# RuihanGao/visual-tactile-synthesis

Hardware: AMD Instinct MI355X
Metric: train_images_per_sec (higher is better)
Workload: dtype f32; 1 GPU; skitG G+D1+D2 train step, 1024x1024 sketch->(RGB,tactile), 4 images/GPU, 64 tactile patches/image, LPIPS/CLIP terms off (no weights offline); global_batch=4, parallelism=dp1, losses_finite=True, hip_graph=True, d2_visualisation_pass=True, train_only=False, full=False

## Files before the change

visual-tactile-synthesis_amd/csrc/vts_conv.hip:

```cpp
#include "vts_conv_kernel.h"

thread_local int t_stat_spl = 0;

namespace {

__global__ __launch_bounds__(256) void conv_split_epilogue_kernel(const ConvK p, int KS) {
  const int co = blockIdx.y, n = blockIdx.z;
  const int64_t oplane = (int64_t)p.OH * p.OW;
  const int64_t o = (int64_t)blockIdx.x * 256 + threadIdx.x;
  if (o >= oplane) return;
  float v = 0.f;
  for (int ks = 0; ks < KS; ++ks) v += p.part[(((int64_t)ks * p.N + n) * p.Cout + co) * oplane + o];
  v += p.bias ? p.bias[co] : 0.f;
  if (p.act_out == VTS_ACT_TANH) v = tanhf(v);
  if (p.dm) {
    const float dsc = p.dmsc ? p.dmsc[n * p.dmC + co] : 1.f, dsh = p.dmsh ? p.dmsh[n * p.dmC + co] : 0.f;
    v *= vts_act_grad(p.dm[n * p.dmns + co * oplane + o] * dsc + dsh, p.dm_act);
  }
  float* ob = p.out + n * p.ons + co * oplane + o;
  *ob = p.accumulate ? *ob + v : v;
}

struct InStatsOut {
  float *scale, *shift, *mean, *rstd;
// ... 143 lines not shown
  VTS_CHECK_ARG(d->stride == 1 || d->stride == 2, "vts_conv4x4: stride %d unsupported", d->stride);
  VTS_CHECK_ARG(d->Cout >= 1, "vts_conv4x4: Cout %d", d->Cout);
  if (d->Cout > 80) {
    for (int c0 = 0; c0 < d->Cout; c0 += 80) {
      vts_conv_desc g = *d;
      const int64_t oplane = (int64_t)d->OH * d->OW;
      g.Cout = d->Cout - c0 < 80 ? d->Cout - c0 : 80;
      g.w = d->w + (int64_t)c0 * d->ws_co;
      g.bias = d->bias ? d->bias + c0 : nullptr;
      g.out = d->out + c0 * oplane;
      if (d->dmask.data) {
        g.dmask.data = d->dmask.data + c0 * oplane;
        g.dmask.scale = d->dmask.scale ? d->dmask.scale + c0 : nullptr;
        g.dmask.shift = d->dmask.shift ? d->dmask.shift + c0 : nullptr;
      }
      const int rc = conv4x4_impl(&g, stream, nullptr, nullptr, StatWs{nullptr, 0});
      if (rc != VTS_OK) return rc;
    }
    return VTS_OK;
  }
  VTS_CHECK_ARG(d->N >= 1 && d->IH >= 1 && d->IW >= 1 && d->OH >= 1 && d->OW >= 1, "vts_conv4x4: bad shape");
  VTS_CHECK_ARG(d->in0.C >= 1 && d->in1.C >= 0, "vts_conv4x4: bad channel counts");
  VTS_CHECK_ARG(d->OH <= d->IH * d->stride + 16 && d->OW <= d->IW * d->stride + 16 && d->pad >= -8 && d->pad <= 8,
                "vts_conv4x4: output %dx%d / pad %d implausible for input %dx%d s%d", d->OH, d->OW, d->pad, d->IH, d->IW, d->stride);
  VTS_CHECK_ARG(d->pad_dx >= -8 && d->pad_dx <= 8 && !(d->transposed && d->stride == 2 && d->pad_dx != 0), "vts_conv4x4: bad pad_dx %d", d->pad_dx);
  if (d->transposed && d->stride == 2) {
    VTS_CHECK_ARG((d->OH + 2 * d->pad - 4) / d->stride + 1 == d->IH && (d->OW + 2 * d->pad - 4) / d->stride + 1 == d->IW && d->pad >= 0,
                  "vts_conv4x4: transposed output %dx%d inconsistent with input %dx%d s%d p%d", d->OH, d->OW, d->IH,
                  d->IW, d->stride, d->pad);
  }
  {
    const int rh0 = vts_conv_head_try(d, (hipStream_t)stream);
    if (rh0 != VTS_ERR_UNSUPPORTED) return rh0;
    static const int use_small = vts_tune_set("VTS_NO_SMALL") ? 0 : 1;
    if (use_small) {
      const int rc = vts_conv_small_try(d, (hipStream_t)stream);
      if (rc != VTS_ERR_UNSUPPORTED) return rc;
    }
  }
  ConvK k;
  k.s0 = d->in0.data; k.sc0 = d->in0.scale; k.sh0 = d->in0.shift; k.ns0 = d->in0.nstride; k.C0 = d->in0.C;
  k.s1 = d->in1.data; k.sc1 = d->in1.scale; k.sh1 = d->in1.shift; k.ns1 = d->in1.nstride;
  k.C1 = d->in1.data ? d->in1.C : 0;
  k.Cin = k.C0 + k.C1;
  k.IH = d->IH; k.IW = d->IW; k.OH = d->OH; k.OW = d->OW; k.Cout = d->Cout; k.pad = d->pad; k.padx = d->pad + d->pad_dx;
  k.w = d->w; k.ws_co = d->ws_co; k.ws_ci = d->ws_ci; k.bias = d->bias;
  k.out = d->out; k.ons = d->out_nstride;
  k.act_in = d->act_in; k.act_out = d->act_out;
  k.dm = d->dmask.data; k.dmsc = d->dmask.scale; k.dmsh = d->dmask.shift; k.dmns = d->dmask.nstride;
  k.dm_act = d->dmask_act; k.dmC = d->dmask.C;
  k.accumulate = d->accumulate;
  k.N = d->N; k.CG = 1; k.cps = 1 << 30; k.part = nullptr; k.tiles_x = 0; k.stat_part = nullptr; k.stat_spl = 0; k.bsum_part = nullptr;
#ifdef VTS_PROFILING
  static const int ablate = vts_tune("VTS_ABLATE", 0);
  k.ablate = ablate;
  k.trace = nullptr;
#endif
  static const int xcd_swizzle = vts_tune("VTS_XCD_SWIZZLE", 1);
  k.xcd_swizzle = xcd_swizzle;
  static const int direct_epi = vts_tune("VTS_DIRECT_EPI", 1);
  k.direct_epi = direct_epi && (int64_t)d->Cout * d->OH * d->OW * 4 < (int64_t)OOB_OFF && (!d->dmask.data || (int64_t)d->dmask.C * d->OH * d->OW * 4 < (int64_t)OOB_OFF);
  k.ident = vts_ident();
  VTS_CHECK_ARG(k.ident, "vts_conv4x4: could not allocate the identity constants");
  {
    const int64_t wfl = (int64_t)(d->Cout - 1) * d->ws_co + (int64_t)(k.Cin - 1) * d->ws_ci + 16;
    VTS_CHECK_ARG(wfl * 4 < (int64_t)OOB_OFF && (int64_t)d->IH * d->IW * 4 < (int64_t)OOB_OFF, "vts_conv4x4: tensor too large for 30-bit buffer offsets");
    k.wbytes = (int)(wfl * 4);
  }
  k.slope_in = vts_slope(d->act_in);
  k.identity_in = (d->act_in == VTS_ACT_NONE && !d->in0.scale && !d->in0.shift && !(d->in1.data && (d->in1.scale || d->in1.shift))) ? 1 : 0;
  hipStream_t st = (hipStream_t)stream;
  const int nr = (d->Cout + 15) / 16;
  const int N = d->N;
  static const int fuse_stats = vts_tune("VTS_FUSE_STATS", 1);
  const bool stats_ok = nd && fused && sw.p && fuse_stats && d->act_out == VTS_ACT_NONE && !d->dmask.data && !d->accumulate &&
                        nd->x == d->out && nd->N == N && nd->C == d->Cout && nd->HW == d->OH * d->OW && nd->nstride == d->out_nstride;
  const bool want_stats = stats_ok && k.direct_epi && sw.floats >= vts_conv4x4_norm_ws_floats(d);
  static const int fuse_bsums = vts_tune("VTS_FUSE_BSUMS", 1);
  const bool bsums_ok = bsums && fused && sw.p && fuse_bsums && d->act_out == VTS_ACT_NONE && d->dmask.data;
  const bool want_bsums = bsums_ok && k.direct_epi && sw.floats >= vts_conv4x4_norm_ws_floats(d);
  {
    int spl = 0;
    const int rc = vts_conv_px_try(d, st, stats_ok ? sw.p : nullptr, (!stats_ok && bsums_ok) ? sw.p : nullptr, sw.floats, &spl);
    if (rc != VTS_ERR_UNSUPPORTED) {
      if (rc == VTS_OK && spl > 0) *fused = 2 + spl;
      return rc;
    }
    const int rt = vts_conv_thin_try(d, st);
    if (rt != VTS_ERR_UNSUPPORTED) return rt;
  }
  {
    int rw, mt;
    full_tile(d->transposed, d->stride, nr, rw, mt);
    const bool ph4 = d->transposed && d->stride == 2;
    const int GH = ph4 ? (d->OH + 1) / 2 : d->OH, GW = ph4 ? (d->OW + 1) / 2 : d->OW;
    const int full_wgs = cdiv(GW, 16 * mt) * cdiv(GH, 4 * rw) * N;
    static const int split_ck = vts_tune("VTS_SPLIT_CK", 8);
    int ck = 4;
    const int nchunks = (k.Cin + 3) / 4;
    static const int small_thr = vts_tune("VTS_SMALL_WGS", 300);
    static const int target_wgs = vts_tune("VTS_TARGET_WGS", 256);
    if (full_wgs < small_thr && (nr > 1 || nchunks >= 8)) {
      const int base = cdiv(GW, 32) * cdiv(GH, 4) * N * nr;
      int KS = target_wgs / base;
      if (KS > nchunks / 2) KS = nchunks / 2;
      if (KS < 1) KS = 1;
      int cps = cdiv(nchunks, KS);
      KS = cdiv(nchunks, cps);
      const int64_t need = (int64_t)KS * N * d->Cout * d->OH * d->OW;
      if (KS > 1 && (!d->ws || d->ws_floats < need)) { KS = 1; cps = nchunks; }
      if (split_ck == 8 && k.Cin >= 32 && cps >= 4 && (cps % 2 == 0 || KS == 1)) { ck = 8; cps = (cps + 1) / 2; }
      k.CG = nr; k.cps = cps; k.part = KS > 1 ? d->ws : nullptr;
      const bool cg_stats = want_stats && KS == 1;
      if (cg_stats) k.stat_part = sw.p;
      const bool cg_bsums = want_bsums && KS == 1;
      if (cg_bsums) k.bsum_part = sw.p;
      int rc;
      if (!d->transposed) rc = d->stride == 2 ? vts_conv_split_m0s2(k, N, st, nr, KS, ck) : vts_conv_split_m0s1(k, N, st, nr, KS, ck);
      else rc = d->stride == 2 ? vts_conv_split_m1s2(k, N, st, nr, KS, ck) : vts_conv_split_m1s1(k, N, st, nr, KS, ck);
      if (rc == VTS_OK && (cg_stats || cg_bsums)) *fused = 2 + t_stat_spl;
      if (rc != VTS_OK || KS == 1) return rc;
      static const int fuse_in = vts_tune("VTS_FUSE_SPLIT_IN", 1);
      if (nd && nd->mode == 0 && fuse_in && (int64_t)d->OH * d->OW <= 4096 && d->act_out == VTS_ACT_NONE && !d->dmask.data && !d->accumulate &&
          nd->x == d->out && nd->N == N && nd->C == d->Cout && nd->HW == d->OH * d->OW && nd->nstride == d->out_nstride) {
        const InStatsOut q{nd->scale, nd->shift, nd->mean_out, nd->rstd_out, nd->eps};
        hipLaunchKernelGGL(conv_split_epilogue_in_kernel, dim3(N * d->Cout), dim3(256), 0, st, k, KS, q);
        VTS_CHECK_LAUNCH("vts_conv4x4 split epilogue + instance norm");
        vts_set_kernel("conv4x4_kernel<%d, %d, 1, 1, 2, %d, false, 0>+ksplit+in", d->transposed ? 1 : 0, d->stride, ck);
        *fused = 1;
        return VTS_OK;
      }
      static const int fuse_inbwd = vts_tune("VTS_FUSE_SPLIT_INBWD", 1);
      if (bsums && in_bwd_ok && fused && fuse_inbwd && (int64_t)d->OH * d->OW <= 4096 && d->act_out == VTS_ACT_NONE && d->dmask.data && d->dmask.scale &&
          d->dmask.shift && d->dmask.C == d->Cout) {
        hipLaunchKernelGGL(conv_split_epilogue_inbwd_kernel, dim3(N * d->Cout), dim3(256), 0, st, k, KS);
        VTS_CHECK_LAUNCH("vts_conv4x4 split epilogue + instance norm backward");
        vts_set_kernel("conv4x4_kernel<%d, %d, 1, 1, 2, %d, false, 0>+ksplit+inbwd", d->transposed ? 1 : 0, d->stride, ck);
        *fused = -1;
        return VTS_OK;
      }
      hipLaunchKernelGGL(conv_split_epilogue_kernel, dim3((unsigned)cdiv64((int64_t)d->OH * d->OW, 256), d->Cout, N), dim3(256), 0, st, k, KS);
      VTS_CHECK_LAUNCH("vts_conv4x4 split epilogue");
      return VTS_OK;
    }
  }
  if (want_stats) k.stat_part = sw.p;
  if (want_bsums) k.bsum_part = sw.p;
  const int rc = dispatch_full(d, k, nr, N, st);
  if (rc != VTS_OK || !(want_stats || want_bsums)) return rc;
  *fused = 2 + t_stat_spl;
  return VTS_OK;
}

static int dispatch_full(const vts_conv_desc* d, const ConvK& k, int nr, int N, hipStream_t st) {
  if (!d->transposed) return d->stride == 2 ? vts_conv_full_m0s2(k, nr, N, st) : vts_conv_full_m0s1(k, nr, N, st);
  return d->stride == 2 ? vts_conv_full_m1s2(k, nr, N, st) : vts_conv_full_m1s1(k, nr, N, st);
}
```

visual-tactile-synthesis_amd/csrc/vts_conv_kernel.h:

```cpp
#pragma once
#include <stdio.h>
#include <stdlib.h>
#include <string.h>

#include "vts_internal.h"

struct ConvK {
  const float *s0, *s1, *sc0, *sh0, *sc1, *sh1;
  int64_t ns0, ns1;
  int C0, C1, Cin;
  int IH, IW, OH, OW, Cout, pad, padx;
  const float* w;
  int ws_co, ws_ci;
  const float* bias;
  float* out;
  int64_t ons;
  int act_in, act_out;
  const float *dm, *dmsc, *dmsh;
  int64_t dmns;
  int dm_act, dmC;
  int accumulate;
  int N, CG, cps;
  float* part;
  const float* ident;
  float slope_in;
  int identity_in;
  int wbytes;
  int xcd_swizzle;
  int direct_epi;
  int tiles_x;
  float* stat_part;
  int stat_spl;
  float* bsum_part;
  unsigned rc_gxy, rc_gx, rc_N, rc_CG, rc_gridx;
#ifdef VTS_PROFILING
  int ablate;
  unsigned long long* trace;
#endif
};

#ifdef VTS_PROFILING
#define VTS_ABL(p, bit) ((p).ablate & (bit))
#else
#define VTS_ABL(p, bit) 0
#endif


extern thread_local int t_stat_spl;

int vts_conv_full_m0s1(const ConvK& k, int nr, int N, hipStream_t st);
int vts_conv_full_m0s2(const ConvK& k, int nr, int N, hipStream_t st);
int vts_conv_full_m1s1(const ConvK& k, int nr, int N, hipStream_t st);
int vts_conv_full_m1s2(const ConvK& k, int nr, int N, hipStream_t st);
int vts_conv_split_m0s1(const ConvK& k, int N, hipStream_t st, int CG, int KS, int ck);
int vts_conv_split_m0s2(const ConvK& k, int N, hipStream_t st, int CG, int KS, int ck);
int vts_conv_split_m1s1(const ConvK& k, int N, hipStream_t st, int CG, int KS, int ck);
int vts_conv_split_m1s2(const ConvK& k, int N, hipStream_t st, int CG, int KS, int ck);

namespace {

typedef __amdgpu_buffer_rsrc_t rsrc_t;
constexpr unsigned OOB_OFF = 0x40000000u;
struct TagT { static constexpr bool value = true; };
struct TagF { static constexpr bool value = false; };
__device__ __forceinline__ float ld_buf(const rsrc_t& rs, unsigned voff) {
  return __builtin_bit_cast(float, __builtin_amdgcn_raw_buffer_load_b32(rs, (int)voff, 0, 0));
}

constexpr int conv_min_waves(int mode, int s, int nr, int rw, int mt, bool run) {
  if (run) return rw * mt * ((mode == 1 && s == 2) ? 4 : 1) * nr * 4 <= 48 ? 3 : 2;
  if (mode == 0 && (nr >= 3 || mt >= 4)) return 1;
  const int acc_regs = rw * mt * ((mode == 1 && s == 2) ? 4 : 1) * nr * 4;
  return acc_regs <= 64 ? 4 : (acc_regs <= 96 ? 3 : 2);
}

__host__ inline unsigned conv_recip(unsigned d) { return d <= 1 ? 0u : (unsigned)((0x100000000ull + d - 1) / d); }
__device__ __forceinline__ int fast_div(int n, int d, unsigned rc) {
  if (rc == 0) return n;
  int q = (int)__umulhi((unsigned)n, rc);
  if (q * d > n) --q;
  return q;
}

template <int MODE, int S, int NR, int RW, int MT, int CK, bool RUN, int STATS>
__global__ __launch_bounds__(256, conv_min_waves(MODE, S, NR, RW, MT, RUN)) void conv4x4_kernel(const ConvK p) {
  constexpr int P = (MODE == 1 && S == 2) ? 4 : 1;
  constexpr int TY = 4 * RW, TX = 16 * MT;
  constexpr int PR = MODE == 0 ? (TY - 1) * S + 4 : (S == 2 ? TY + 2 : TY + 3);
  constexpr int PC = MODE == 0 ? (TX - 1) * S + 4 : (S == 2 ? TX + 2 : TX + 3);
  constexpr int PCP = PC + 1;
  constexpr int COP = (NR % 2 == 1) ? NR * 16 : NR * 16 + 16;
  static_assert(CK % 4 == 0 && CK >= 4 && CK <= 16, "staging maps wave w to the input channels w, w + 4, ... of the chunk");
  constexpr int CKW = CK / 4;
  constexpr int REM = PC % 64;
  constexpr int NCM = PC / 64 + ((REM > 16) ? 1 : 0);
  constexpr int PCM = (REM > 16) ? PC : (PC / 64) * 64;
  constexpr int TW = PC - PCM;
  constexpr int NROWS = CK * PR;
  constexpr int NPV = PR * NCM > 0 ? PR * NCM : 1;
  constexpr int NTV = (NROWS * TW + 255) / 256 > 0 ? (NROWS * TW + 255) / 256 : 1;
  constexpr int NWV = CKW * NR;
  constexpr int EC = (P == 4) ? 2 * TX : TX;
  constexpr int EPL = TY * EC + 1;
  constexpr int PATCH_FLOATS = CK * PR * PCP, W_FLOATS = CK * 16 * COP;
  constexpr int OUT_FLOATS = (NR == 1 && RW == 1 && MT == 2) ? 16 * EPL : 0;
  constexpr int LDS_FLOATS = (PATCH_FLOATS + W_FLOATS) > OUT_FLOATS ? (PATCH_FLOATS + W_FLOATS) : OUT_FLOATS;

  __shared__ float lds[LDS_FLOATS];
  __shared__ float lds_stat[STATS ? 4 * NR * 16 * 3 : 1];
  float* lds_patch = lds;
  float* lds_w = lds + PATCH_FLOATS;

  const int tid = threadIdx.x, lane = tid & 63;
#ifdef VTS_PROFILING
  const int trace_wg = blockIdx.x + gridDim.x * (blockIdx.y + gridDim.y * blockIdx.z);
  auto stamp = [&](int i) {
    if (p.trace && tid == 0) p.trace[(int64_t)trace_wg * 8 + i] = i == 0 ? (unsigned long long)__builtin_amdgcn_s_getreg((4 << 0) | (0 << 6) | (31 << 11)) | ((unsigned long long)__builtin_amdgcn_s_getreg((20 << 0) | (0 << 6) | (31 << 11)) << 32) : __builtin_amdgcn_s_memrealtime();
  };
#else
  auto stamp = [](int) {};
#endif
  stamp(0);
  stamp(1);
  const int wave = __builtin_amdgcn_readfirstlane(tid >> 6);
  const int m16 = lane & 15, kq = lane >> 4;
  int bx = blockIdx.x, by = blockIdx.y, bz = blockIdx.z;
  if (p.xcd_swizzle) {
    const int gx = gridDim.x, gy = gridDim.y, nwg = gx * gy * (int)gridDim.z;
    const int lin = bx + gx * (by + gy * bz);
    const int q = nwg >> 3, r = nwg & 7, xcd = lin & 7, idx = lin >> 3;
    const int lin2 = xcd * q + min(xcd, r) + idx;
    bz = fast_div(lin2, gx * gy, p.rc_gxy);
    const int rem = lin2 - bz * (gx * gy);
    by = fast_div(rem, gx, p.rc_gx);
    bx = rem - by * gx;
  }
  const int bzn = fast_div(bz, p.N, p.rc_N), n = bz - bzn * p.N;
  const int ks = fast_div(bzn, p.CG, p.rc_CG), cg = bzn - ks * p.CG;
  const int co0 = cg * NR * 16;
  const int tile_begin = RUN ? fast_div(bx * p.tiles_x, (int)gridDim.x, p.rc_gridx) : bx;
  const int tile_end = RUN ? fast_div((bx + 1) * p.tiles_x, (int)gridDim.x, p.rc_gridx) : bx + 1;
  const int ty0 = by * TY;
  const int podd = p.pad & 1;

  int iy0;
  if (MODE == 0) iy0 = ty0 * S - p.pad;
  else if (S == 2) iy0 = ty0 + (p.pad >> 1) - 1;
  else iy0 = ty0 + p.pad - 3;

  int aoff[P];
  if (MODE == 0) {
    aoff[0] = (wave * RW * S) * PCP + m16 * S + kq;
  } else if (S == 2) {
#pragma unroll
    for (int ph = 0; ph < P; ++ph) {
      const int dpy = (ph >> 1) & podd, dpx = (ph & 1) & podd;
      aoff[ph] = (wave * RW + dpy + 1 - (kq >> 1)) * PCP + m16 + dpx + 1 - (kq & 1);
    }
  } else {
    aoff[0] = (wave * RW + 3) * PCP + m16 + 3 - kq;
  }

  f32x4 acc[RW][MT][P][NR];
#pragma unroll
  for (int r = 0; r < RW; ++r)
#pragma unroll
    for (int mt = 0; mt < MT; ++mt)
#pragma unroll
      for (int ph = 0; ph < P; ++ph)
#pragma unroll
        for (int nr = 0; nr < NR; ++nr) acc[r][mt][ph][nr] = (f32x4){0.f, 0.f, 0.f, 0.f};

  const int64_t plane = (int64_t)p.IH * p.IW;
  const int nchunks = (p.Cin + CK - 1) / CK;
  const int chunk_begin = ks * p.cps;
  const int chunk_end = min(nchunks, (ks + 1) * p.cps);

  constexpr int TPR = TW > 0 ? 64 / TW : 1;
  static_assert(TW == 0 || PR <= TPR, "one tail load covers all patch rows");
  float pv[CKW][NPV], tv[CKW];
  f32x4 wv[NWV];
#pragma unroll
  for (int h = 0; h < CKW; ++h) {
    tv[h] = 0.f;
#pragma unroll
    for (int i = 0; i < NPV; ++i) pv[h][i] = 0.f;
  }
#pragma unroll
  for (int i = 0; i < NWV; ++i) wv[i] = (f32x4){1.f, 1.f, 1.f, 1.f};

  const int iplane = p.IH * p.IW;
  const float* sb0 = p.s0 + n * p.ns0;
  const float* sb1 = p.s1 + n * p.ns1;
  const unsigned row0 = (unsigned)(iy0 * p.IW * 4), rstep = (unsigned)(p.IW * 4);
  unsigned vo_m[NCM > 0 ? NCM : 1];
  int colw[NCM > 0 ? NCM : 1];
#pragma unroll
  for (int cm = 0; cm < NCM; ++cm) {
    const int col = cm * 64 + lane;
    vo_m[cm] = OOB_OFF;
    colw[cm] = col < PCM ? col : PC;
  }
  unsigned vo_t = OOB_OFF;
  int dst_t = PC;
  const int r_t = lane / (TW > 0 ? TW : 1), c_t = lane - r_t * (TW > 0 ? TW : 1);
  if (TW > 0) dst_t = r_t < PR ? r_t * PCP + PCM + c_t : PC;
  auto set_tile = [&](int tile) {
    const int tx0 = tile * TX;
    int ix0;
    if (MODE == 0) ix0 = tx0 * S - p.padx;
    else if (S == 2) ix0 = tx0 + (p.pad >> 1) - 1;
    else ix0 = tx0 + p.padx - 3;
#pragma unroll
    for (int cm = 0; cm < NCM; ++cm) {
      const int col = cm * 64 + lane, ix = ix0 + col;
      vo_m[cm] = (col < PCM && ix >= 0 && ix < p.IW) ? (unsigned)ix * 4u : OOB_OFF;
    }
    if (TW > 0) {
      const int ix = ix0 + PCM + c_t;
      vo_t = (r_t < PR && ix >= 0 && ix < p.IW) ? (unsigned)(r_t * p.IW + ix) * 4u : OOB_OFF;
    }
  };
  float wsc[CKW], wsh[CKW];
  unsigned cur_nrec[CKW];
#pragma unroll
  for (int h = 0; h < CKW; ++h) {
    wsc[h] = 1.f;
    wsh[h] = 0.f;
    cur_nrec[h] = 0;
  }

  constexpr int NCO = NR * 16;
  unsigned wvo[NWV];
  int wc[NWV], wld[NWV][4];
#pragma unroll
  for (int e = 0; e < NWV; ++e) {
    const int u = tid + e * 256;
    const int co = u % NCO, rest = u / NCO;
    const int ky = rest & 3, c = rest >> 2;
    wc[e] = c;
    wvo[e] = co0 + co < p.Cout ? (unsigned)((co0 + co) * p.ws_co + c * p.ws_ci + ky * 4) * 4u : OOB_OFF;
#pragma unroll
    for (int kx = 0; kx < 4; ++kx) {
      int slot = ky * 4 + kx;
      if (MODE == 1 && S == 2) slot = ((((ky + p.pad) & 1) * 2 + ((kx + p.pad) & 1)) * 4) + (ky >> 1) * 2 + (kx >> 1);
      wld[e][kx] = (c * 16 + slot) * COP + co;
    }
  }
  const rsrc_t wrs = __builtin_amdgcn_make_buffer_rsrc((void*)p.w, 0, p.wbytes, 0x00020000);

  auto opaque_zero = []() {
    int z = 0;
    asm volatile("" : "+s"(z));
    return z;
  };

  auto load_chunk = [&](int chunk, bool with_w) {
    const int cbase = chunk * CK;
#pragma unroll
    for (int h = 0; h < CKW; ++h) {
      const int cic = cbase + wave + 4 * h + opaque_zero();
      {
        const int ccl = min(cic, p.Cin - 1);
        const bool first = ccl < p.C0;
        const int cl = first ? ccl : ccl - p.C0;
        const float* scp = first ? p.sc0 : p.sc1;
        const float* shp = first ? p.sh0 : p.sh1;
        const int aidx = n * (first ? p.C0 : p.C1) + cl;
        const bool hsc = scp != nullptr, hsh = shp != nullptr;
        wsc[h] = (hsc ? scp : p.ident)[hsc ? aidx : 0];
        wsh[h] = (hsh ? shp : p.ident)[hsh ? aidx : 1];
      }
      const bool cok = cic < p.Cin;
      const int cc = cok ? cic : 0;
      const bool first = cc < p.C0;
      const float* base = (first ? sb0 : sb1) + (int64_t)(first ? cc : cc - p.C0) * iplane;
      cur_nrec[h] = cok ? (unsigned)iplane * 4u : 0u;
      const rsrc_t rs = __builtin_amdgcn_make_buffer_rsrc((void*)base, 0, (int)cur_nrec[h], 0x00020000);
#pragma unroll
      for (int r = 0; r < PR; ++r)
#pragma unroll
        for (int cm = 0; cm < NCM; ++cm) pv[h][r * NCM + cm] = ld_buf(rs, vo_m[cm] + row0 + r * rstep);
      if (TW > 0) tv[h] = ld_buf(rs, vo_t + row0);
    }
    if (with_w) {
      const int wsoff = cbase * p.ws_ci * 4;
#pragma unroll
      for (int e = 0; e < NWV; ++e)
        wv[e] = __builtin_bit_cast(f32x4, __builtin_amdgcn_raw_buffer_load_b128(wrs, (int)(cbase + wc[e] < p.Cin ? wvo[e] : OOB_OFF), wsoff, 0));
    }
  };

  auto finish = [&](float x, float sc, float sh, bool inside) -> float {
    const float t = fmaf(x, sc, sh);
    const float a = fmaxf(t, 0.f) + p.slope_in * fminf(t, 0.f);
    return inside ? a : 0.f;
  };

  auto store_patch = [&](auto plain_tag) {
    constexpr bool PLAIN = decltype(plain_tag)::value;
#pragma unroll
    for (int h = 0; h < CKW; ++h) {
      float* dst = lds_patch + (wave + 4 * h) * PR * PCP;
#pragma unroll
      for (int r = 0; r < PR; ++r)
#pragma unroll
        for (int cm = 0; cm < NCM; ++cm) {
          float v = pv[h][r * NCM + cm];
          if (!PLAIN) v = finish(v, wsc[h], wsh[h], vo_m[cm] + row0 + r * rstep < cur_nrec[h]);
          dst[r * PCP + colw[cm]] = v;
        }
      if (TW > 0) {
        float v = tv[h];
// ... 39 lines not shown
              for (int j = 0; j < 4; ++j) {
                const float v = j < nv ? a[j] : 0.f;
                sum += v;
                sq = fmaf(v, v, sq);
              }
              cnt += (float)max(nv, 0);
            }
        sum += __shfl_xor(sum, 16, 64);
        sq += __shfl_xor(sq, 16, 64);
        cnt += __shfl_xor(cnt, 16, 64);
        sum += __shfl_xor(sum, 32, 64);
        sq += __shfl_xor(sq, 32, 64);
        cnt += __shfl_xor(cnt, 32, 64);
        if (kq == 0) {
          const float mean = sum / fmaxf(cnt, 1.f);
          float* q = lds_stat + (wave * NR * 16 + nr * 16 + m16) * 3;
          q[0] = mean;
          q[1] = fmaxf(sq - sum * mean, 0.f);
          q[2] = cnt;
        }
      }
      __syncthreads();
      if (tid < NR * 16 && co0 + tid < p.Cout) {
        float cnt = 0.f, wm = 0.f;
#pragma unroll
        for (int w = 0; w < 4; ++w) {
          const float* q = lds_stat + (w * NR * 16 + tid) * 3;
          cnt += q[2];
          wm = fmaf(q[2], q[0], wm);
        }
        const float mean = wm / fmaxf(cnt, 1.f);
        float m2 = 0.f;
#pragma unroll
        for (int w = 0; w < 4; ++w) {
          const float* q = lds_stat + (w * NR * 16 + tid) * 3;
          const float d = q[0] - mean;
          m2 += q[1] + q[2] * d * d;
        }
        const int co = co0 + tid;
        float* o = p.stat_part + (((int64_t)n * p.Cout + co) * p.stat_spl + slot) * 3;
        o[0] = mean + (p.bias ? p.bias[co] : 0.f);
        o[1] = m2;
        o[2] = cnt;
      }
      __syncthreads();
    }
    float bs1 = 0.f, bs2 = 0.f;
    auto emit = [&](int co, int y, int x, float bias, float dsc, float dsh, f32x4 v) {
      const bool ok = co < p.Cout && y < p.OH && x < p.OW;
      const bool full = ok && x + 4 <= p.OW;
      const unsigned off = (unsigned)((co * (int)oplane + y * p.OW + x) * 4);
      const unsigned vo = full ? off : OOB_OFF;
#pragma unroll
      for (int j = 0; j < 4; ++j) {
        float t = v[j] + bias;
        if (p.act_out == VTS_ACT_TANH) t = tanhf(t);
        v[j] = t;
      }
      const f32x4 base = v;
      f32x4 tn = {0.f, 0.f, 0.f, 0.f};
      if (p.dm) {
        const f32x4 d = __builtin_bit_cast(f32x4, __builtin_amdgcn_raw_buffer_load_b128(drs, (int)vo, 0, 0));
#pragma unroll
        for (int j = 0; j < 4; ++j) {
          tn[j] = d[j] * dsc + dsh;
          v[j] *= vts_act_grad(tn[j], p.dm_act);
        }
      }
      if (p.accumulate) {
        const f32x4 q = __builtin_bit_cast(f32x4, __builtin_amdgcn_raw_buffer_load_b128(ors, (int)vo, 0, 0));
#pragma unroll
        for (int j = 0; j < 4; ++j) v[j] += q[j];
      }
      if (STATS == 2 && full) {
#pragma unroll
        for (int j = 0; j < 4; ++j) {
          bs1 += v[j];
          bs2 = fmaf(v[j], tn[j], bs2);
        }
      }
      __builtin_amdgcn_raw_buffer_store_b128(__builtin_bit_cast(__attribute__((ext_vector_type(4))) unsigned, v), ors, (int)vo, 0, 0);
      if (ok && !full) {
        float* ob = p.out + n * p.ons + co * oplane + (int64_t)y * p.OW + x;
        const float* db = p.dm ? p.dm + n * p.dmns + co * oplane + (int64_t)y * p.OW + x : nullptr;
        for (int j = 0; j < p.OW - x; ++j) {
          float t = base[j];
          const float tnj = db ? db[j] * dsc + dsh : 0.f;
          if (db) t *= vts_act_grad(tnj, p.dm_act);
          const float fin = p.accumulate ? ob[j] + t : t;
          ob[j] = fin;
          if (STATS == 2) {
            bs1 += fin;
            bs2 = fmaf(fin, tnj, bs2);
          }
        }
      }
    };
#pragma unroll
    for (int nr = 0; nr < NR; ++nr) {
      const int co = co0 + nr * 16 + m16;
      const int coc = min(co, p.Cout - 1);
      const float bias = p.bias ? p.bias[coc] : 0.f;
      const float dsc = (p.dm && p.dmsc) ? p.dmsc[n * p.dmC + coc] : 1.f, dsh = (p.dm && p.dmsh) ? p.dmsh[n * p.dmC + coc] : 0.f;
#pragma unroll
      for (int r = 0; r < RW; ++r)
#pragma unroll
        for (int mt = 0; mt < MT; ++mt) {
          const int gy = ty0e + wave * RW + r, gx = tx0 + mt * 16 + kq * 4;
          if (P == 1) {
            emit(co, gy, gx, bias, dsc, dsh, acc[r][mt][0][nr]);
          } else {
#pragma unroll
            for (int py = 0; py < 2; ++py) {
              const f32x4 a = acc[r][mt][P == 4 ? py * 2 : 0][nr], b = acc[r][mt][P == 4 ? py * 2 + 1 : 0][nr];
              emit(co, gy * 2 + py, gx * 2, bias, dsc, dsh, (f32x4){a[0], b[0], a[1], b[1]});
              emit(co, gy * 2 + py, gx * 2 + 4, bias, dsc, dsh, (f32x4){a[2], b[2], a[3], b[3]});
            }
          }
#pragma unroll
          for (int ph = 0; ph < P; ++ph) acc[r][mt][ph][nr] = (f32x4){0.f, 0.f, 0.f, 0.f};
        }
      if (STATS == 2) {
        bs1 += __shfl_xor(bs1, 16, 64);
        bs2 += __shfl_xor(bs2, 16, 64);
        bs1 += __shfl_xor(bs1, 32, 64);
        bs2 += __shfl_xor(bs2, 32, 64);
        if (kq == 0) {
          float* q = lds_stat + (wave * NR * 16 + nr * 16 + m16) * 3;
          q[0] = bs1;
          q[1] = bs2;
        }
        bs1 = 0.f;
        bs2 = 0.f;
      }
    }
    if (STATS == 2) {
      __syncthreads();
      if (tid < NR * 16 && co0 + tid < p.Cout) {
        float s1 = 0.f, s2 = 0.f;
#pragma unroll
        for (int w = 0; w < 4; ++w) {
          const float* q = lds_stat + (w * NR * 16 + tid) * 3;
          s1 += q[0];
          s2 += q[1];
        }
        const int slot = by * p.tiles_x + tx0 / TX;
        float* o = p.bsum_part + (((int64_t)n * p.Cout + co0 + tid) * p.stat_spl + slot) * 2;
        o[0] = s1;
        o[1] = s2;
      }
      __syncthreads();
    }
  };

  const int nch = chunk_end - chunk_begin;
  const int units = nch > 0 ? nch * (tile_end - tile_begin) : 0;
  const bool reload_w = !RUN || nch > 1;
  stamp(2);
  if (units > 0) {
    set_tile(tile_begin);
    if (!VTS_ABL(p, 1)) load_chunk(chunk_begin, true);
    stamp(3);
    store_chunk(true);
  }
  __syncthreads();
  stamp(4);
  int chunk = chunk_begin, tile = tile_begin;
  for (int u = 0; u < units; ++u) {
    const bool more = u + 1 < units;
    int chunk_n = chunk + 1, tile_n = tile;
    if (chunk_n == chunk_end) {
      chunk_n = chunk_begin;
      tile_n = tile + 1;
    }
    if (more) {
      if (RUN && tile_n != tile) set_tile(tile_n);
      if (!VTS_ABL(p, 1)) load_chunk(chunk_n, reload_w);
    }
    const int cvalid = VTS_ABL(p, 2) ? 0 : min(CK, p.Cin - chunk * CK);
    {
      constexpr int NA = RW * MT;
      auto rd = [&](int c, int g, float (&av)[NA], float (&bv)[NR]) {
        const float* pp = lds_patch + c * PR * PCP;
        const float* ww = lds_w + c * 16 * COP + kq * COP + m16;
#pragma unroll
        for (int nr = 0; nr < NR; ++nr) bv[nr] = ww[g * 4 * COP + nr * 16];
#pragma unroll
        for (int r = 0; r < RW; ++r)
#pragma unroll
          for (int mt = 0; mt < MT; ++mt) {
            if (MODE == 1 && S == 2) av[r * MT + mt] = pp[aoff[P == 4 ? g : 0] + r * PCP + mt * 16];
            else if (MODE == 0) av[r * MT + mt] = pp[aoff[0] + (r * S + g) * PCP + mt * 16 * S];
            else av[r * MT + mt] = pp[aoff[0] + (r - g) * PCP + mt * 16];
          }
      };
      auto mm = [&](int g, const float (&av)[NA], const float (&bv)[NR]) {
#pragma unroll
        for (int r = 0; r < RW; ++r)
#pragma unroll
          for (int mt = 0; mt < MT; ++mt)
#pragma unroll
            for (int nr = 0; nr < NR; ++nr)
              acc[r][mt][P == 4 ? g : 0][nr] = __builtin_amdgcn_mfma_f32_16x16x4f32(av[r * MT + mt], bv[nr], acc[r][mt][P == 4 ? g : 0][nr], 0, 0, 0);
      };
#ifndef VTS_DEEP_MAX
#define VTS_DEEP_MAX 4
#endif
      if constexpr (NA * NR <= VTS_DEEP_MAX) {
        float av[4][NA], bv[4][NR];
        if (cvalid > 0) {
          rd(0, 0, av[0], bv[0]);
          rd(0, 1, av[1], bv[1]);
          rd(0, 2, av[2], bv[2]);
        }
        for (int c = 0; c < cvalid; ++c) {
          const int cn = min(c + 1, CK - 1);
          rd(c, 3, av[3], bv[3]);
          __builtin_amdgcn_sched_barrier(0);
          mm(0, av[0], bv[0]);
          __builtin_amdgcn_sched_barrier(0);
          rd(cn, 0, av[0], bv[0]);
          __builtin_amdgcn_sched_barrier(0);
          mm(1, av[1], bv[1]);
          __builtin_amdgcn_sched_barrier(0);
          rd(cn, 1, av[1], bv[1]);
          __builtin_amdgcn_sched_barrier(0);
          mm(2, av[2], bv[2]);
          __builtin_amdgcn_sched_barrier(0);
          rd(cn, 2, av[2], bv[2]);
          __builtin_amdgcn_sched_barrier(0);
          mm(3, av[3], bv[3]);
          __builtin_amdgcn_sched_barrier(0);
        }
      } else {
        float ax[NA], bx[NR], ay[NA], by_[NR];
        if (cvalid > 0) rd(0, 0, ax, bx);
        for (int c = 0; c < cvalid; ++c) {
          rd(c, 1, ay, by_);
          __builtin_amdgcn_sched_barrier(0);
          mm(0, ax, bx);
          __builtin_amdgcn_sched_barrier(0);
          rd(c, 2, ax, bx);
          __builtin_amdgcn_sched_barrier(0);
          mm(1, ay, by_);
          __builtin_amdgcn_sched_barrier(0);
          rd(c, 3, ay, by_);
          __builtin_amdgcn_sched_barrier(0);
          mm(2, ax, bx);
          __builtin_amdgcn_sched_barrier(0);
          if (c + 1 < cvalid) rd(c + 1, 0, ax, bx);
          __builtin_amdgcn_sched_barrier(0);
          mm(3, ay, by_);
          __builtin_amdgcn_sched_barrier(0);
        }
      }
    }
    if (u == 0) stamp(5);
    if (RUN && direct && tile_n != tile) {
      if (VTS_ABL(p, 4)) {
        if (acc[0][0][0][0][0] == 123.456f) p.out[0] = 1.f;
      } else {
        epilogue_direct(tile * TX, ty0 + opaque_zero());
      }
    }
    __syncthreads();
    if (more) {
      store_chunk(reload_w);
      __syncthreads();
    }
    chunk = chunk_n;
    tile = tile_n;
  }
  stamp(6);
  if (RUN) return;
  const int tx0 = tile_begin * TX;
  if (direct) {
    if (!VTS_ABL(p, 4)) epilogue_direct(tx0, ty0);
    else if (acc[0][0][0][0][0] == 123.456f) p.out[0] = 1.f;
    stamp(7);
    return;
  }
  if constexpr (!(NR == 1 && RW == 1 && MT == 2)) return;

  if (VTS_ABL(p, 4)) {
    if (acc[0][0][0][0][0] == 123.456f) p.out[0] = 1.f;
    return;
  }
  constexpr int PY = (P == 4) ? 2 : 1;
  const int oy0 = (P == 4) ? ty0 * 2 : ty0, ox0 = (P == 4) ? tx0 * 2 : tx0;
  float* so = lds;
  const bool vec_ok = ((p.OW & 3) == 0) && ((p.ons & 3) == 0) && ((reinterpret_cast<uintptr_t>(p.out) & 15) == 0) &&
                      (!p.part || (reinterpret_cast<uintptr_t>(p.part) & 15) == 0) &&
                      (!p.dm || (((p.dmns & 3) == 0) && ((reinterpret_cast<uintptr_t>(p.dm) & 15) == 0)));
#pragma unroll
  for (int nr = 0; nr < NR; ++nr) {
#pragma unroll
    for (int py = 0; py < PY; ++py) {
#pragma unroll
      for (int r = 0; r < RW; ++r)
#pragma unroll
        for (int mt = 0; mt < MT; ++mt)
#pragma unroll
          for (int px = 0; px < (P == 4 ? 2 : 1); ++px) {
            const int ph = py * 2 + px;
            const int row = wave * RW + r;
#pragma unroll
            for (int j = 0; j < 4; ++j) {
              const int xl = mt * 16 + kq * 4 + j;
              const int col = (P == 4) ? xl * 2 + px : xl;
              so[m16 * EPL + row * EC + col] = acc[r][mt][P == 4 ? ph : 0][nr][j];
            }
          }
      __syncthreads();
      for (int idx = tid; idx < 16 * TY * (EC / 4); idx += 256) {
        const int c16 = idx / (TY * (EC / 4));
        const int rem = idx - c16 * (TY * (EC / 4));
        const int row = rem / (EC / 4), x4 = (rem - row * (EC / 4)) * 4;
        const int co = co0 + nr * 16 + c16;
        const int y = (P == 4) ? oy0 + row * 2 + py : oy0 + row;
        const int x = ox0 + x4;
        if (co >= p.Cout || y >= p.OH || x >= p.OW) continue;
        const float* sp = so + c16 * EPL + row * EC + x4;
        float v[4] = {sp[0], sp[1], sp[2], sp[3]};
        const int64_t o = (int64_t)y * p.OW + x;
        const int nvalid = min(4, p.OW - x);
        if (p.part) {
          float* pb = p.part + (((int64_t)ks * p.N + n) * p.Cout + co) * oplane + o;
          if (vec_ok && nvalid == 4) {
            *reinterpret_cast<f32x4*>(pb) = (f32x4){v[0], v[1], v[2], v[3]};
          } else {
#pragma unroll
            for (int j = 0; j < 4; ++j)
              if (j < nvalid) pb[j] = v[j];
          }
          continue;
        }
        const float bias = p.bias ? p.bias[co] : 0.f;
        float* ob = p.out + n * p.ons + co * oplane + o;
        float dv[4] = {1.f, 1.f, 1.f, 1.f}, prev[4] = {0.f, 0.f, 0.f, 0.f};
        const bool vec = vec_ok && nvalid == 4;
        if (p.dm) {
          const float dsc = p.dmsc ? p.dmsc[n * p.dmC + co] : 1.f, dsh = p.dmsh ? p.dmsh[n * p.dmC + co] : 0.f;
          const float* db = p.dm + n * p.dmns + co * oplane + o;
          if (vec) {
            const f32x4 t = *reinterpret_cast<const f32x4*>(db);
#pragma unroll
            for (int j = 0; j < 4; ++j) dv[j] = vts_act_grad(t[j] * dsc + dsh, p.dm_act);
          } else {
#pragma unroll
            for (int j = 0; j < 4; ++j)
              if (j < nvalid) dv[j] = vts_act_grad(db[j] * dsc + dsh, p.dm_act);
          }
        }
        if (p.accumulate) {
          if (vec) {
            const f32x4 t = *reinterpret_cast<const f32x4*>(ob);
#pragma unroll
            for (int j = 0; j < 4; ++j) prev[j] = t[j];
          } else {
#pragma unroll
            for (int j = 0; j < 4; ++j)
              if (j < nvalid) prev[j] = ob[j];
          }
        }
#pragma unroll
        for (int j = 0; j < 4; ++j) {
          float t = v[j] + bias;
          if (p.act_out == VTS_ACT_TANH) t = tanhf(t);
          v[j] = t * dv[j] + prev[j];
        }
        if (vec) {
          *reinterpret_cast<f32x4*>(ob) = (f32x4){v[0], v[1], v[2], v[3]};
        } else {
#pragma unroll
          for (int j = 0; j < 4; ++j)
            if (j < nvalid) ob[j] = v[j];
        }
      }
      __syncthreads();
    }
  }
}

inline bool vts_prefer_mt3(const ConvK& k, bool phases4, int mt_default) {
  static const int on = vts_tune("VTS_MT3", 1);
  const int GW = phases4 ? (k.OW + 1) / 2 : k.OW;
  const int c3 = cdiv(GW, 48) * 48, cd = cdiv(GW, 16 * mt_default) * 16 * mt_default;
  return on && c3 * 100 < cd * 93;
}

template <int MODE, int S, int NR, int RW, int MT, int CK>
int launch(const ConvK& k0, int N, hipStream_t st, int CG = 1, int KS = 1) {
  constexpr int P = (MODE == 1 && S == 2) ? 4 : 1;
  ConvK k = k0;
  const int GH = P == 4 ? (k.OH + 1) / 2 : k.OH, GW = P == 4 ? (k.OW + 1) / 2 : k.OW;
  const int tiles_x = cdiv(GW, 16 * MT), tiles_y = cdiv(GH, 4 * RW);
  k.tiles_x = tiles_x;
  k.stat_spl = tiles_x * tiles_y;
  t_stat_spl = k.stat_spl;
  static const int run_force = vts_tune("VTS_TILE_RUN", 0);
  static const int run_wgs = vts_tune("VTS_TILE_RUN_WGS", 2048);
  static const int run_max_chunks = vts_tune("VTS_TILE_RUN_CHUNKS", 4);
  int run = 1;
  if (NR <= 2 && !k.part && k.direct_epi && KS == 1) {
    const int64_t total = (int64_t)tiles_x * tiles_y * N * CG;
    const int nchunks = (k.Cin + CK - 1) / CK;
    if (run_force > 0) run = run_force;
    else if (nchunks <= run_max_chunks) run = (int)(total / run_wgs);
    if (run > tiles_x) run = tiles_x;
    if (run < 1) run = 1;
  }
  if (CK != 4) run = 1;
  dim3 grid(cdiv(tiles_x, run), tiles_y, N * CG * KS);
  k.rc_gxy = conv_recip(grid.x * grid.y); k.rc_gx = k.rc_gridx = conv_recip(grid.x);
  k.rc_N = conv_recip((unsigned)k.N); k.rc_CG = conv_recip((unsigned)k.CG);
  if (!(NR == 1 && RW == 1 && MT == 2) && (k.part || !k.direct_epi)) {
    vts_set_error("vts_conv4x4: this tile instance has no LDS epilogue (VTS_DIRECT_EPI=0 / output beyond 30-bit offsets)");
    return VTS_ERR_UNSUPPORTED;
  }
#ifdef VTS_PROFILING
  static const char* trace_path = getenv("VTS_CONV_TRACE");
  unsigned long long* trace_dev = nullptr;
  const int64_t trace_wgs = (int64_t)grid.x * grid.y * grid.z;
  if (trace_path) {
    char tag[64];
    snprintf(tag, sizeof tag, "%d,%d,%d,%d,%d", MODE, S, NR, RW, MT);
    const char* want = getenv("VTS_CONV_TRACE_KERNEL");
    if (!want || strcmp(want, tag) == 0) {
      if (hipMalloc(&trace_dev, trace_wgs * 64) != hipSuccess) trace_dev = nullptr;
      if (trace_dev) (void)hipMemsetAsync(trace_dev, 0, trace_wgs * 64, st);
    }
  }
  k.trace = trace_dev;
#endif
  constexpr bool RUNI = (NR <= 2) && CK == 4;
  if (CK != 4) run = 1;
  if (k.stat_part) {
    if (run > 1) hipLaunchKernelGGL((conv4x4_kernel<MODE, S, NR, RW, MT, CK, RUNI, 1>), grid, dim3(256), 0, st, k);
    else hipLaunchKernelGGL((conv4x4_kernel<MODE, S, NR, RW, MT, CK, false, 1>), grid, dim3(256), 0, st, k);
  } else if (k.bsum_part) {
    if (run > 1) hipLaunchKernelGGL((conv4x4_kernel<MODE, S, NR, RW, MT, CK, RUNI, 2>), grid, dim3(256), 0, st, k);
    else hipLaunchKernelGGL((conv4x4_kernel<MODE, S, NR, RW, MT, CK, false, 2>), grid, dim3(256), 0, st, k);
  } else {
    if (run > 1) hipLaunchKernelGGL((conv4x4_kernel<MODE, S, NR, RW, MT, CK, RUNI, 0>), grid, dim3(256), 0, st, k);
    else hipLaunchKernelGGL((conv4x4_kernel<MODE, S, NR, RW, MT, CK, false, 0>), grid, dim3(256), 0, st, k);
  }
  vts_set_kernel("conv4x4_kernel<%d, %d, %d, %d, %d, %d, %s, %s>%s", MODE, S, NR, RW, MT, CK, (run > 1 && NR <= 2) ? "true" : "false",
                 k.stat_part ? "1" : (k.bsum_part ? "2" : "0"), KS > 1 ? "+ksplit" : (CG > 1 ? "+coutsplit" : ""));
  VTS_CHECK_LAUNCH("vts_conv4x4");
#ifdef VTS_PROFILING
  if (trace_dev) {
    (void)hipStreamSynchronize(st);
    unsigned long long* h = (unsigned long long*)malloc(trace_wgs * 64);
    (void)hipMemcpy(h, trace_dev, trace_wgs * 64, hipMemcpyDeviceToHost);
    FILE* f = fopen(trace_path, "a");
    if (f) {
      fprintf(f, "# conv4x4_kernel<%d,%d,%d,%d,%d> run %d grid %u %u %u Cin %d Cout %d OH %d OW %d\n", MODE, S, NR, RW, MT, run, grid.x, grid.y, grid.z, k.Cin, k.Cout, k.OH, k.OW);
      for (int64_t w = 0; w < trace_wgs; ++w) {
        fprintf(f, "%lld %llx", (long long)w, h[w * 8]);
        for (int i = 1; i < 8; ++i) fprintf(f, " %llu", h[w * 8 + i]);
        fprintf(f, "\n");
      }
      fclose(f);
    }
    free(h);
    (void)hipFree(trace_dev);
  }
#endif
  return VTS_OK;
}



}
```

Baseline: 762.5 images/s.

## Route transposed stride-2 convs through split-bf16x3 MFMA kernel

Adds a new conv4x4 kernel variant for transposed stride-2 convolutions with two output-channel groups. It splits each f32 input and weight into three bf16 parts and accumulates six cross-product MFMA bf16 passes, which emulates f32 accuracy on the bf16 matrix cores in place of the existing f32 path. Operands are staged in LDS as packed bf16x8 with 8-channel chunks, and the next chunk is software-prefetched. The cost is extra split/convert work, a larger LDS footprint and a fixed occupancy of 2 waves, and the results are no longer bit-identical to the f32 path.

```diff
diff --git a/visual-tactile-synthesis_amd/csrc/vts_conv.hip b/visual-tactile-synthesis_amd/csrc/vts_conv.hip
--- a/visual-tactile-synthesis_amd/csrc/vts_conv.hip
+++ b/visual-tactile-synthesis_amd/csrc/vts_conv.hip
@@ -319,7 +319,14 @@
   return VTS_OK;
 }
 
+static bool conv_route_bf3(const vts_conv_desc* d, const ConvK& k, int nr) {
+  static const int on = vts_tune("VTS_CONV_BF3", 1);
+  if (!on || k.Cin < 8) return false;
+  return d->transposed && d->stride == 2 && nr == 2;
+}
+
 static int dispatch_full(const vts_conv_desc* d, const ConvK& k, int nr, int N, hipStream_t st) {
+  if (conv_route_bf3(d, k, nr)) return vts_conv_full_bf3_m1s2(k, nr, N, st);
   if (!d->transposed) return d->stride == 2 ? vts_conv_full_m0s2(k, nr, N, st) : vts_conv_full_m0s1(k, nr, N, st);
   return d->stride == 2 ? vts_conv_full_m1s2(k, nr, N, st) : vts_conv_full_m1s1(k, nr, N, st);
 }
diff --git a/visual-tactile-synthesis_amd/csrc/vts_conv_bf3_m1s2.hip b/visual-tactile-synthesis_amd/csrc/vts_conv_bf3_m1s2.hip
--- /dev/null
+++ b/visual-tactile-synthesis_amd/csrc/vts_conv_bf3_m1s2.hip
@@ -0,0 +1,11 @@
+#include "vts_conv_kernel.h"
+
+
+int vts_conv_full_bf3_m1s2(const ConvK& k, int nr, int N, hipStream_t st) {
+  switch (nr) {
+    case 2: return launch<1, 2, 2, 1, 2, 8, true>(k, N, st);
+    default:
+      vts_set_error("vts_conv4x4: no split-bf16 instance for the transposed stride-2 operator with %d output-channel groups", nr);
+      return VTS_ERR_UNSUPPORTED;
+  }
+}
diff --git a/visual-tactile-synthesis_amd/csrc/vts_conv_kernel.h b/visual-tactile-synthesis_amd/csrc/vts_conv_kernel.h
--- a/visual-tactile-synthesis_amd/csrc/vts_conv_kernel.h
+++ b/visual-tactile-synthesis_amd/csrc/vts_conv_kernel.h
@@ -56,6 +56,7 @@
 int vts_conv_split_m0s2(const ConvK& k, int N, hipStream_t st, int CG, int KS, int ck);
 int vts_conv_split_m1s1(const ConvK& k, int N, hipStream_t st, int CG, int KS, int ck);
 int vts_conv_split_m1s2(const ConvK& k, int N, hipStream_t st, int CG, int KS, int ck);
+int vts_conv_full_bf3_m1s2(const ConvK& k, int nr, int N, hipStream_t st);
 
 namespace {
 
@@ -67,7 +68,26 @@
   return __builtin_bit_cast(float, __builtin_amdgcn_raw_buffer_load_b32(rs, (int)voff, 0, 0));
 }
 
-constexpr int conv_min_waves(int mode, int s, int nr, int rw, int mt, bool run) {
+typedef __bf16 bf16x8 __attribute__((ext_vector_type(8)));
+struct Split3 {
+  bf16x8 p[3];
+};
+__device__ __forceinline__ Split3 split8(const float (&x)[8]) {
+  Split3 s;
+#pragma unroll
+  for (int i = 0; i < 8; ++i) {
+    const __bf16 h = (__bf16)x[i];
+    const float r1 = x[i] - (float)h;
+    const __bf16 m = (__bf16)r1;
+    s.p[0][i] = h;
+    s.p[1][i] = m;
+    s.p[2][i] = (__bf16)(r1 - (float)m);
+  }
+  return s;
+}
+
+constexpr int conv_min_waves(int mode, int s, int nr, int rw, int mt, bool run, bool bf3 = false) {
+  if (bf3) return 2;
   if (run) return rw * mt * ((mode == 1 && s == 2) ? 4 : 1) * nr * 4 <= 48 ? 3 : 2;
   if (mode == 0 && (nr >= 3 || mt >= 4)) return 1;
   const int acc_regs = rw * mt * ((mode == 1 && s == 2) ? 4 : 1) * nr * 4;
@@ -82,8 +102,8 @@
   return q;
 }
 
-template <int MODE, int S, int NR, int RW, int MT, int CK, bool RUN, int STATS>
-__global__ __launch_bounds__(256, conv_min_waves(MODE, S, NR, RW, MT, RUN)) void conv4x4_kernel(const ConvK p) {
+template <int MODE, int S, int NR, int RW, int MT, int CK, bool RUN, int STATS, bool BF3 = false>
+__global__ __launch_bounds__(256, conv_min_waves(MODE, S, NR, RW, MT, RUN, BF3)) void conv4x4_kernel(const ConvK p) {
   constexpr int P = (MODE == 1 && S == 2) ? 4 : 1;
   constexpr int TY = 4 * RW, TX = 16 * MT;
   constexpr int PR = MODE == 0 ? (TY - 1) * S + 4 : (S == 2 ? TY + 2 : TY + 3);
@@ -104,9 +124,13 @@
   constexpr int EPL = TY * EC + 1;
   constexpr int PATCH_FLOATS = CK * PR * PCP, W_FLOATS = CK * 16 * COP;
   constexpr int OUT_FLOATS = (NR == 1 && RW == 1 && MT == 2) ? 16 * EPL : 0;
-  constexpr int LDS_FLOATS = (PATCH_FLOATS + W_FLOATS) > OUT_FLOATS ? (PATCH_FLOATS + W_FLOATS) : OUT_FLOATS;
-
-  __shared__ float lds[LDS_FLOATS];
+  static_assert(!BF3 || (CK == 8 && !RUN), "split-bf16 instances: 8-channel chunks, one tile per workgroup");
+  constexpr int BF_PLANE = PR * PC * 16, BF_WPLANE = 16 * NR * 16 * 16;
+  constexpr int BF_FLOATS = (3 * BF_PLANE + 3 * BF_WPLANE) / 4;
+  constexpr int MAIN_FLOATS = BF3 ? BF_FLOATS : PATCH_FLOATS + W_FLOATS;
+  constexpr int LDS_FLOATS = MAIN_FLOATS > OUT_FLOATS ? MAIN_FLOATS : OUT_FLOATS;
+
+  __shared__ alignas(BF3 ? 16 : alignof(float)) float lds[LDS_FLOATS];
   __shared__ float lds_stat[STATS ? 4 * NR * 16 * 3 : 1];
   float* lds_patch = lds;
   float* lds_w = lds + PATCH_FLOATS;
@@ -148,17 +172,18 @@
   else if (S == 2) iy0 = ty0 + (p.pad >> 1) - 1;
   else iy0 = ty0 + p.pad - 3;
 
+  constexpr int APITCH = BF3 ? PC : PCP;
   int aoff[P];
   if (MODE == 0) {
-    aoff[0] = (wave * RW * S) * PCP + m16 * S + kq;
+    aoff[0] = (wave * RW * S) * APITCH + m16 * S + kq;
   } else if (S == 2) {
 #pragma unroll
     for (int ph = 0; ph < P; ++ph) {
       const int dpy = (ph >> 1) & podd, dpx = (ph & 1) & podd;
-      aoff[ph] = (wave * RW + dpy + 1 - (kq >> 1)) * PCP + m16 + dpx + 1 - (kq & 1);
+      aoff[ph] = (wave * RW + dpy + 1 - (kq >> 1)) * APITCH + m16 + dpx + 1 - (kq & 1);
     }
   } else {
-    aoff[0] = (wave * RW + 3) * PCP + m16 + 3 - kq;
+    aoff[0] = (wave * RW + 3) * APITCH + m16 + 3 - kq;
   }
 
   f32x4 acc[RW][MT][P][NR];
@@ -504,6 +529,183 @@
       __syncthreads();
     }
   };
+
+  if constexpr (BF3) {
+    char* const lb = reinterpret_cast<char*>(lds);
+    constexpr int NA = RW * MT;
+    constexpr int NPOS = (PR * PC + 255) / 256;
+    constexpr int NWU = (4 * NCO + 255) / 256;
+    int ix0;
+    {
+      const int tx0 = tile_begin * TX;
+      if (MODE == 0) ix0 = tx0 * S - p.padx;
+      else if (S == 2) ix0 = tx0 + (p.pad >> 1) - 1;
+      else ix0 = tx0 + p.padx - 3;
+    }
+    unsigned vpos[NPOS];
+#pragma unroll
+    for (int i = 0; i < NPOS; ++i) {
+      const int pos = tid + 256 * i, r = pos / PC, c = pos - r * PC;
+      const int iy = iy0 + r, ix = ix0 + c;
+      vpos[i] = (pos < PR * PC && iy >= 0 && iy < p.IH && ix >= 0 && ix < p.IW) ? (unsigned)(iy * p.IW + ix) * 4u : OOB_OFF;
+    }
+    unsigned wvo[NWU];
+#pragma unroll
+    for (int e = 0; e < NWU; ++e) {
+      const int u = tid + 256 * e, co = u % NCO, ky = u / NCO;
+      wvo[e] = (u < 4 * NCO && co0 + co < p.Cout) ? (unsigned)((co0 + co) * p.ws_co + ky * 4) * 4u : OOB_OFF;
+    }
+    float xv[NPOS][8], csc[8], csh[8];
+    unsigned cnrec[8];
+    f32x4 wq[NWU][8];
+    auto load_bf = [&](int chunk) __attribute__((always_inline)) {
+      const int cbase = chunk * 8;
+#pragma unroll
+      for (int j = 0; j < 8; ++j) {
+        const int cic = cbase + j + opaque_zero();
+        {
+          const int ccl = min(cic, p.Cin - 1);
+          const bool first = ccl < p.C0;
+          const int cl = first ? ccl : ccl - p.C0;
+          const float* scp = first ? p.sc0 : p.sc1;
+          const float* shp = first ? p.sh0 : p.sh1;
+          const int aidx = n * (first ? p.C0 : p.C1) + cl;
+          const bool hsc = scp != nullptr, hsh = shp != nullptr;
+          csc[j] = (hsc ? scp : p.ident)[hsc ? aidx : 0];
+          csh[j] = (hsh ? shp : p.ident)[hsh ? aidx : 1];
+        }
+        const bool cok = cic < p.Cin;
+        const int cc = cok ? cic : 0;
+        const bool first = cc < p.C0;
+        const float* base = (first ? sb0 : sb1) + (int64_t)(first ? cc : cc - p.C0) * iplane;
+        cnrec[j] = cok ? (unsigned)iplane * 4u : 0u;
+        const rsrc_t rs = __builtin_amdgcn_make_buffer_rsrc((void*)base, 0, (int)cnrec[j], 0x00020000);
+#pragma unroll
+        for (int i = 0; i < NPOS; ++i) xv[i][j] = ld_buf(rs, vpos[i]);
+#pragma unroll
+        for (int e = 0; e < NWU; ++e)
+          wq[e][j] = __builtin_bit_cast(f32x4, __builtin_amdgcn_raw_buffer_load_b128(wrs, (int)(cok ? wvo[e] : OOB_OFF), cic * p.ws_ci * 4, 0));
+      }
+    };
+    auto store_bf = [&](auto plain_tag) __attribute__((always_inline)) {
+      constexpr bool PLAIN = decltype(plain_tag)::value;
+#pragma unroll
+      for (int i = 0; i < NPOS; ++i) {
+        const int pos = tid + 256 * i;
+        if (pos < PR * PC) {
+          float x[8];
+#pragma unroll
+          for (int j = 0; j < 8; ++j) {
+            x[j] = xv[i][j];
+            if (!PLAIN) {
+              const float t = fmaf(x[j], csc[j], csh[j]);
+              const float a = fmaxf(t, 0.f) + p.slope_in * fminf(t, 0.f);
+              x[j] = vpos[i] < cnrec[j] ? a : 0.f;
+            }
+          }
+          const Split3 sp = split8(x);
+#pragma unroll
+          for (int k = 0; k < 3; ++k) *reinterpret_cast<bf16x8*>(lb + k * BF_PLANE + pos * 16) = sp.p[k];
+        }
+      }
+#pragma unroll
+      for (int e = 0; e < NWU; ++e) {
+        const int u = tid + 256 * e, co = u % NCO, ky = u / NCO;
+        if (u < 4 * NCO) {
+#pragma unroll
+          for (int kx = 0; kx < 4; ++kx) {
+            int slot = ky * 4 + kx;
+            if (MODE == 1 && S == 2) slot = ((((ky + p.pad) & 1) * 2 + ((kx + p.pad) & 1)) * 4) + (ky >> 1) * 2 + (kx >> 1);
+            float x[8];
+#pragma unroll
+            for (int j = 0; j < 8; ++j) x[j] = wq[e][j][kx];
+            const Split3 sp = split8(x);
+#pragma unroll
+            for (int k = 0; k < 3; ++k) *reinterpret_cast<bf16x8*>(lb + 3 * BF_PLANE + k * BF_WPLANE + (slot * NCO + co) * 16) = sp.p[k];
+          }
+        }
+      }
+    };
+    auto store_chunk_bf = [&]() __attribute__((always_inline)) {
+      if (p.identity_in) store_bf(TagT());
+      else store_bf(TagF());
+    };
+    auto rdb = [&](int g, bf16x8 (&a)[NA][3], bf16x8 (&b)[NR][3]) __attribute__((always_inline)) {
+#pragma unroll
+      for (int nr = 0; nr < NR; ++nr)
+#pragma unroll
+        for (int k = 0; k < 3; ++k) b[nr][k] = *reinterpret_cast<const bf16x8*>(lb + 3 * BF_PLANE + k * BF_WPLANE + ((g * 4 + kq) * NCO + nr * 16 + m16) * 16);
+#pragma unroll
+      for (int r = 0; r < RW; ++r)
+#pragma unroll
+        for (int mt = 0; mt < MT; ++mt) {
+          int pos;
+          if (MODE == 1 && S == 2) pos = aoff[P == 4 ? g : 0] + r * PC + mt * 16;
+          else if (MODE == 0) pos = aoff[0] + (r * S + g) * PC + mt * 16 * S;
+          else pos = aoff[0] + (r - g) * PC + mt * 16;
+#pragma unroll
+          for (int k = 0; k < 3; ++k) a[r * MT + mt][k] = *reinterpret_cast<const bf16x8*>(lb + k * BF_PLANE + pos * 16);
+        }
+    };
+    auto mmb = [&](int g, const bf16x8 (&a)[NA][3], const bf16x8 (&b)[NR][3]) __attribute__((always_inline)) {
+      constexpr int PA[6] = {2, 1, 0, 1, 0, 0}, PB[6] = {0, 1, 2, 0, 1, 0};
+#pragma unroll
+      for (int q = 0; q < 6; ++q)
+#pragma unroll
+        for (int r = 0; r < RW; ++r)
+#pragma unroll
+          for (int mt = 0; mt < MT; ++mt)
+#pragma unroll
+            for (int nr = 0; nr < NR; ++nr)
+              acc[r][mt][P == 4 ? g : 0][nr] =
+                  __builtin_amdgcn_mfma_f32_16x16x32_bf16(a[r * MT + mt][PA[q]], b[nr][PB[q]], acc[r][mt][P == 4 ? g : 0][nr], 0, 0, 0);
+    };
+    const int nch = chunk_end - chunk_begin;
+    stamp(2);
+    if (nch > 0) {
+      if (!VTS_ABL(p, 1)) load_bf(chunk_begin);
+      stamp(3);
+      store_chunk_bf();
+    }
+    __syncthreads();
+    stamp(4);
+    for (int u = 0; u < nch; ++u) {
+      const bool more = u + 1 < nch;
+      if (more && !VTS_ABL(p, 1)) load_bf(chunk_begin + u + 1);
+      if (!VTS_ABL(p, 2)) {
+        bf16x8 ax[NA][3], bx[NR][3], ay[NA][3], by_[NR][3];
+        rdb(0, ax, bx);
+        rdb(1, ay, by_);
+        __builtin_amdgcn_sched_barrier(0);
+        mmb(0, ax, bx);
+        __builtin_amdgcn_sched_barrier(0);
+        rdb(2, ax, bx);
+        __builtin_amdgcn_sched_barrier(0);
+        mmb(1, ay, by_);
+        __builtin_amdgcn_sched_barrier(0);
+        rdb(3, ay, by_);
+        __builtin_amdgcn_sched_barrier(0);
+        mmb(2, ax, bx);
+        __builtin_amdgcn_sched_barrier(0);
+        mmb(3, ay, by_);
+        __builtin_amdgcn_sched_barrier(0);
+      }
+      if (u == 0) stamp(5);
+      __syncthreads();
+      if (more) {
+        store_chunk_bf();
+        __syncthreads();
+      }
+    }
+    stamp(6);
+    const int tx0 = tile_begin * TX;
+    if (direct) {
+      if (!VTS_ABL(p, 4)) epilogue_direct(tx0, ty0);
+      else if (acc[0][0][0][0][0] == 123.456f) p.out[0] = 1.f;
+      stamp(7);
+    }
+    return;
+  }
 
   const int nch = chunk_end - chunk_begin;
   const int units = nch > 0 ? nch * (tile_end - tile_begin) : 0;
@@ -741,7 +943,7 @@
   return on && c3 * 100 < cd * 93;
 }
 
-template <int MODE, int S, int NR, int RW, int MT, int CK>
+template <int MODE, int S, int NR, int RW, int MT, int CK, bool BF3 = false>
 int launch(const ConvK& k0, int N, hipStream_t st, int CG = 1, int KS = 1) {
   constexpr int P = (MODE == 1 && S == 2) ? 4 : 1;
   ConvK k = k0;
@@ -766,7 +968,7 @@
   dim3 grid(cdiv(tiles_x, run), tiles_y, N * CG * KS);
   k.rc_gxy = conv_recip(grid.x * grid.y); k.rc_gx = k.rc_gridx = conv_recip(grid.x);
   k.rc_N = conv_recip((unsigned)k.N); k.rc_CG = conv_recip((unsigned)k.CG);
-  if (!(NR == 1 && RW == 1 && MT == 2) && (k.part || !k.direct_epi)) {
+  if ((BF3 || !(NR == 1 && RW == 1 && MT == 2)) && (k.part || !k.direct_epi)) {
     vts_set_error("vts_conv4x4: this tile instance has no LDS epilogue (VTS_DIRECT_EPI=0 / output beyond 30-bit offsets)");
     return VTS_ERR_UNSUPPORTED;
   }
@@ -787,7 +989,11 @@
 #endif
   constexpr bool RUNI = (NR <= 2) && CK == 4;
   if (CK != 4) run = 1;
-  if (k.stat_part) {
+  if constexpr (BF3) {
+    if (k.stat_part) hipLaunchKernelGGL((conv4x4_kernel<MODE, S, NR, RW, MT, CK, false, 1, true>), grid, dim3(256), 0, st, k);
+    else if (k.bsum_part) hipLaunchKernelGGL((conv4x4_kernel<MODE, S, NR, RW, MT, CK, false, 2, true>), grid, dim3(256), 0, st, k);
+    else hipLaunchKernelGGL((conv4x4_kernel<MODE, S, NR, RW, MT, CK, false, 0, true>), grid, dim3(256), 0, st, k);
+  } else if (k.stat_part) {
     if (run > 1) hipLaunchKernelGGL((conv4x4_kernel<MODE, S, NR, RW, MT, CK, RUNI, 1>), grid, dim3(256), 0, st, k);
     else hipLaunchKernelGGL((conv4x4_kernel<MODE, S, NR, RW, MT, CK, false, 1>), grid, dim3(256), 0, st, k);
   } else if (k.bsum_part) {
@@ -797,8 +1003,8 @@
     if (run > 1) hipLaunchKernelGGL((conv4x4_kernel<MODE, S, NR, RW, MT, CK, RUNI, 0>), grid, dim3(256), 0, st, k);
     else hipLaunchKernelGGL((conv4x4_kernel<MODE, S, NR, RW, MT, CK, false, 0>), grid, dim3(256), 0, st, k);
   }
-  vts_set_kernel("conv4x4_kernel<%d, %d, %d, %d, %d, %d, %s, %s>%s", MODE, S, NR, RW, MT, CK, (run > 1 && NR <= 2) ? "true" : "false",
-                 k.stat_part ? "1" : (k.bsum_part ? "2" : "0"), KS > 1 ? "+ksplit" : (CG > 1 ? "+coutsplit" : ""));
+  vts_set_kernel("conv4x4_kernel<%d, %d, %d, %d, %d, %d, %s, %s>%s%s", MODE, S, NR, RW, MT, CK, (run > 1 && NR <= 2) ? "true" : "false",
+                 k.stat_part ? "1" : (k.bsum_part ? "2" : "0"), KS > 1 ? "+ksplit" : (CG > 1 ? "+coutsplit" : ""), BF3 ? "+bf3" : "");
   VTS_CHECK_LAUNCH("vts_conv4x4");
 #ifdef VTS_PROFILING
   if (trace_dev) {
```

After: 759.8 images/s, median of 2. About the same (-0.4%).
